# speechbrain/speechbrain

Measured on AMD Instinct MI355X. Metric: audio-sec/s decoded (node), Conformer-L beam=10, higher is better.
Workload: dtype f32

## Files before the change

speechbrain_amd/csrc/ctc_prefix.hip:

```cpp
#include "common.h"
#include "internal.h"

namespace {

constexpr float kNeg = sbk::kCtcNeg;
constexpr int kNegE = -(1 << 20);
constexpr int kHead = 24;

struct BF {
  float mg, mb;
  int eg, eb;
};

__device__ __forceinline__ float bf_log(float m, int e) {
  if (!(m > 0.0f)) return kNeg;
  const double v = ((double)e + (double)log2f(m)) * 0.69314718055994530942;
  return v < (double)kNeg ? kNeg : (float)v;
}
__device__ __forceinline__ void bf_exp(float x, float* m, int* e) {
  if (!(x > -1e19f)) {
    *m = 0.0f;
    *e = kNegE;
    return;
  }
  const double y = (double)x * 1.44269504088896340736;
  const double ip = floor(y);
  *m = exp2f((float)(y - ip));
  *e = (int)ip;
}

constexpr int kSeg = 32;
__device__ __host__ __forceinline__ int nseg_of(int T) { return (T + kSeg - 1) / kSeg; }
__device__ __host__ __forceinline__ int beam_pitch(int beam) { return 16 * ((beam + 15) / 16); }

template <typename Row>
__device__ __forceinline__ void build_segment_tables(Row row, int T, int lane, float* __restrict__ sg,
                                                     float* __restrict__ sb, int* __restrict__ se, int bp) {
  const int nseg = nseg_of(T);
  for (int s0 = 0; s0 < nseg; s0 += 2) {
    const int seg = s0 + (lane >> 5);
    const int t = seg * kSeg + (lane & 31);
    BF v{0.0f, 0.0f, kNegE, kNegE};
    if (seg < nseg && t < T) v = row(t);
    int e = max(v.mg > 0.0f ? v.eg : kNegE, v.mb > 0.0f ? v.eb : kNegE);
#pragma unroll
    for (int m = 16; m >= 1; m >>= 1) e = max(e, sbk::shfl_xor(e, m));
    if (seg < nseg && t < T) {
      sg[(size_t)t * bp] = sbk::fast_ldexp(v.mg, v.eg - e);
      sb[t] = sbk::fast_ldexp(v.mb, v.eb - e);
    }
    if (seg < nseg && (lane & 31) == 0) se[(size_t)seg * bp] = e;
  }
}

__global__ void __launch_bounds__(256) ctc_emissions_kernel(float* __restrict__ x, float* __restrict__ xb_log,
                                                            const int32_t* __restrict__ enc_len, int T, int V, int blank, int ldp) {
  const int b = blockIdx.y, t = blockIdx.x;
  float* row = x + ((size_t)b * T + t) * ldp;
  const bool pad = t >= enc_len[b];
  if (threadIdx.x == 0) xb_log[b * T + t] = pad ? (blank == 0 ? 0.0f : kNeg) : row[blank];
  __syncthreads();
  for (int c = threadIdx.x; c < V; c += 256) row[c] = pad ? (c == 0 ? 1.0f : 0.0f) : expf(row[c]);
}

__global__ void __launch_bounds__(256) ctc_init_kernel(const float* __restrict__ xb_log, BF* __restrict__ st,
                                                       float* __restrict__ sg, float* __restrict__ sb,
                                                       int* __restrict__ se, float* __restrict__ psi_prev, int T,
                                                       int beam) {
  SBK_DYN_LDS(float, cum);
  const int b = blockIdx.x;
  const int nseg = nseg_of(T);
  if (threadIdx.x == 0) {
    float c = 0.0f;
    for (int t = 0; t < T; ++t) {
      c += xb_log[b * T + t];
      cum[t] = c;
    }
  }
  __syncthreads();
  for (int t = threadIdx.x; t < T; t += 256) {
    BF v;
    bf_exp(cum[t], &v.mg, &v.eg);
    v.mb = v.mg;
    v.eb = v.eg;
    for (int j = 0; j < beam; ++j) st[((size_t)b * beam + j) * T + t] = v;
  }
  if (threadIdx.x < beam) psi_prev[b * beam + threadIdx.x] = 0.0f;
  __syncthreads();
  const int lane = threadIdx.x & 63, wave = threadIdx.x >> 6;
  for (int j = wave; j < beam; j += 4) {
    const size_t n = (size_t)b * beam + j;
    const BF* rowp = st + n * T;
    const int bp = beam_pitch(beam);
    build_segment_tables([&](int t) { return rowp[t]; }, T, lane, sg + (size_t)b * T * bp + j, sb + n * T,
                         se + (size_t)b * nseg * bp + j, bp);
  }
}

struct CtcStepArgs {
  const int32_t* last_tok;
  const int32_t* enc_len;
  int B, T, V, beam, prefix_len, blank, eos;
  float weight;
  int eos_floor;
  int use_eos_threshold;
  float eos_threshold, minus_inf;
  const int32_t* step_ptr;
  int min_steps;
  const int32_t* utt_min;
  int utt_beam, step;
  const int32_t* win;
  int window;
  int ldp;
};
__device__ __forceinline__ void ctc_frame_range(int prefix_len, int T, const int32_t* win, int window, int* start, int* end) {
// ... 109 lines not shown
      for (int q = 0; q < CH; ++q) cur[k][q] = nxt[k][q];
    if (cb + CH < u_end) fetch(nxt, cb + CH);
#pragma unroll
    for (int q = 0; q < CH; ++q) {
      const float4* row = reinterpret_cast<const float4*>(tab + (size_t)min(cb + q, u_end - 1) * BP);
      float g[NV * 4];
#pragma unroll
      for (int v = 0; v < NV; ++v) {
        const float4 t4 = row[v];
        g[4 * v] = t4.x; g[4 * v + 1] = t4.y; g[4 * v + 2] = t4.z; g[4 * v + 3] = t4.w;
      }
#pragma unroll
      for (int k = 0; k < TPT; ++k)
#pragma unroll
        for (int j = 0; j < NB; ++j) part[k][j] = fmaf(g[j], cur[k][q], part[k][j]);
    }
    if (((cb + CH) % kSeg) == 0 || cb + CH >= u_end) {
      const int* es = segs + (cb / kSeg) * BP;
#pragma unroll
      for (int k = 0; k < TPT; ++k)
#pragma unroll
        for (int j = 0; j < NB; ++j) {
          const int kx = sbk::frexp_exp(part[k][j]);
          const int ep = part[k][j] > 0.0f ? es[j] + kx : kNegE;
          const float mp = sbk::fast_ldexp(part[k][j], -kx);
          const int P2 = max(Eps[k][j], ep);
          mps[k][j] = sbk::fast_ldexp(mps[k][j], Eps[k][j] - P2) + sbk::fast_ldexp(mp, ep - P2);
          Eps[k][j] = P2;
          part[k][j] = 0.0f;
        }
    }
  }
#pragma unroll
  for (int k = 0; k < TPT; ++k) {
    if (!c_ok[k]) continue;
#pragma unroll
    for (int j = 0; j < NB; ++j) {
      if (j0 + j < a.beam) {
        const int n = b * a.beam + j0 + j;
        float psi = bf_log(mps[k][j], Eps[k][j]);
        if (c[k] == a.eos) {
          const BF s = st[(size_t)n * T + last_frame];
          psi = bf_log(s.mg, s.eg);
        }
        if (c[k] == a.blank && a.eos != a.blank) psi = kNeg;
        psi_out[(size_t)n * V + c[k]] = psi;
      }
    }
  }
}

__global__ void __launch_bounds__(64) ctc_same_token_kernel(CtcStepArgs a, const float* __restrict__ P,
                                                            const BF* __restrict__ st, const float* __restrict__ sb,
                                                            const int* __restrict__ se, float* __restrict__ psi_out) {
  const int n = blockIdx.x, lane = threadIdx.x;
  if (a.step_ptr) a.prefix_len = a.step_ptr[0];
  const int b = n / a.beam, c = a.last_tok[n];
  const int T = a.T, V = a.V, nseg = nseg_of(T);
  if (c == a.eos || c == a.blank || c < 0 || c >= V) return;
  int start, end;
  ctc_frame_range(a.prefix_len, T, a.win, a.window, &start, &end);
  end = ctc_clip_to_length(end, a.blank, a.enc_len[b]);
  const float* Pb = P + (size_t)b * T * a.ldp;
  float m = 0.0f;
  int E = kNegE;
  if (lane == 0 && a.prefix_len == 0 && start == 1 && Pb[c] > 0.0f) {
    m = Pb[c];
    E = 0;
  }
  for (int u = start - 1 + lane; u < end - 1; u += 64) {
    const float bt = a.win ? st[(size_t)n * T + u].mb : sb[(size_t)n * T + u];
    const float term = bt * Pb[(size_t)(u + 1) * a.ldp + c];
    const int k = sbk::frexp_exp(term);
    const int eb = a.win ? st[(size_t)n * T + u].eb : se[((size_t)b * nseg + u / kSeg) * beam_pitch(a.beam) + n % a.beam];
    const int et = term > 0.0f ? eb + k : kNegE;
    const float mt = sbk::fast_ldexp(term, -k);
    const int E2 = max(E, et);
    m = sbk::fast_ldexp(m, E - E2) + sbk::fast_ldexp(mt, et - E2);
    E = E2;
  }
  int Emax = E;
#pragma unroll
  for (int k = 32; k >= 1; k >>= 1) Emax = max(Emax, sbk::shfl_xor(Emax, k));
  float v = sbk::fast_ldexp(m, E - Emax);
  v = sbk::wave_sum(v);
  if (lane == 0) psi_out[(size_t)n * V + c] = bf_log(v, Emax);
}

__global__ void __launch_bounds__(256) ctc_combine_kernel(CtcStepArgs a, const float* __restrict__ am,
                                                          const float* __restrict__ am_max,
                                                          const float* __restrict__ psi,
                                                          const float* __restrict__ psi_prev, float* __restrict__ comb,
                                                          const float* __restrict__ extra) {
  const int n = blockIdx.y;
  const int c = blockIdx.x * 256 + threadIdx.x;
  if (c >= a.V) return;
  float v = am[(size_t)n * a.V + c];
  if (c == a.eos) {
    const int step = a.step_ptr ? a.step_ptr[0] : a.step;
    const bool floor = a.utt_min ? step < a.utt_min[n / a.utt_beam] : (a.step_ptr ? step < a.min_steps : a.eos_floor);
    if (floor) v = a.minus_inf;
    if (a.use_eos_threshold && !(v > a.eos_threshold * am_max[n])) v = a.minus_inf;
  }
  if (extra) v = sbk::add_rn(v, extra[(size_t)n * a.V + c]);
  if (c == a.blank) v = kNeg;
  comb[(size_t)n * a.V + c] = sbk::score_ctc(v, psi[(size_t)n * a.V + c], psi_prev[n], a.weight);
}

struct AMap {
  float a, c, d, v0, v1;
  int ea, ec, ed, e0, e1;
};
struct AState {
  float nb, bl;
  int e;
};
__device__ __forceinline__ int clamp_e(int e) { return max(e, kNegE); }
__device__ __forceinline__ void norm1(float& x, int& e) {
  const int k = sbk::frexp_exp(x);
  x = sbk::fast_ldexp(x, -k);
  e = x > 0.0f ? clamp_e(e + k) : kNegE;
}
__device__ __forceinline__ void norm2(float& x, float& y, int& e) {
  const float m = fmaxf(x, y);
  const int k = sbk::frexp_exp(m);
  x = sbk::fast_ldexp(x, -k);
  y = sbk::fast_ldexp(y, -k);
  e = m > 0.0f ? e + k : kNegE;
}
__device__ __forceinline__ void bf_add(float& x, int& ex, float y, int ey) {
  const int ax = x > 0.0f ? ex : kNegE, ay = y > 0.0f ? ey : kNegE;
  const int E = max(ax, ay);
// ... 36 lines not shown
  return r;
}
__device__ __forceinline__ AMap frame_map(float pc, float pb, float mphi, int ephi) {
  AMap m;
  m.a = pc;
  m.ea = 0;
  norm1(m.a, m.ea);
  m.c = pb;
  m.ec = 0;
  norm1(m.c, m.ec);
  m.d = m.c;
  m.ed = m.ec;
  m.v0 = m.a * mphi;
  m.e0 = clamp_e(m.ea + ephi);
  norm1(m.v0, m.e0);
  m.v1 = 0.0f;
  m.e1 = kNegE;
  return m;
}
__device__ __forceinline__ AMap identity_map() { return AMap{1.0f, 0.0f, 1.0f, 0.0f, 0.0f, 0, kNegE, 0, kNegE, kNegE}; }
__device__ __forceinline__ AMap shfl_up_map(const AMap& m, int delta, int lane) {
  const int src = max(lane - delta, 0);
  AMap r;
  r.a = sbk::shfl(m.a, src);
  r.c = sbk::shfl(m.c, src);
  r.d = sbk::shfl(m.d, src);
  r.v0 = sbk::shfl(m.v0, src);
  r.v1 = sbk::shfl(m.v1, src);
  r.ea = sbk::shfl(m.ea, src);
  r.ec = sbk::shfl(m.ec, src);
  r.ed = sbk::shfl(m.ed, src);
  r.e0 = sbk::shfl(m.e0, src);
  r.e1 = sbk::shfl(m.e1, src);
  return r;
}

struct CtcAdvArgs {
  const float* P;
  const BF* st_old;
  const float* psi;
  const int32_t* parent;
  const int32_t* token;
  const int32_t* parent_last_tok;
  BF* st_new;
  float* sg_new;
  float* sb_new;
  int* se_new;
  float* psi_prev_new;
  int n_bh, T, V, beam, prefix_len, blank;
  const int32_t* step_ptr;
  const int32_t* win;
  int window;
  int ldp;
};

__global__ void __launch_bounds__(64) ctc_advance_kernel(CtcAdvArgs a) {
  SBK_DYN_LDS(float, lds);
  if (a.step_ptr) a.prefix_len = a.step_ptr[0];
  const int T = a.T;
  float* pc = lds;
  float* pb = pc + T;
  float* mph = pb + T;
  int* eph = reinterpret_cast<int*>(mph + T);
  float* onb = reinterpret_cast<float*>(eph + T);
  float* obl = onb + T;
  int* oe = reinterpret_cast<int*>(obl + T);
  const int n = blockIdx.x, lane = threadIdx.x;
  const int b = n / a.beam, p = a.parent[n], c = a.token[n];
  const bool same = a.parent_last_tok[p] == c;
  const float* Pb = a.P + (size_t)b * T * a.ldp;
  for (int tb = 0; tb < T; tb += 256) {
    float vpc[4], vpb[4];
    BF vs[4];
#pragma unroll
    for (int u = 0; u < 4; ++u) {
      const int t = min(tb + u * 64 + lane, T - 1);
      vpc[u] = Pb[(size_t)t * a.ldp + c];
      vpb[u] = Pb[(size_t)t * a.ldp + a.blank];
      vs[u] = a.st_old[(size_t)p * T + t];
    }
#pragma unroll
    for (int u = 0; u < 4; ++u) {
      const int t = tb + u * 64 + lane;
      if (t < T) {
        pc[t] = vpc[u];
        pb[t] = vpb[u];
        mph[t] = same ? vs[u].mb : vs[u].mg;
        eph[t] = same ? vs[u].eb : vs[u].eg;
      }
    }
  }
  __syncthreads();
  {
    int start, end;
    ctc_frame_range(a.prefix_len, T, a.win, a.window, &start, &end);
    const bool first = a.prefix_len == 0 && pc[0] > 0.0f;
    AState r0{first ? pc[0] : 0.0f, 0.0f, first ? 0 : kNegE};
    norm2(r0.nb, r0.bl, r0.e);
    const AState zero{0.0f, 0.0f, kNegE};
    const AState s0 = start == 1 ? r0 : zero;
    for (int t = lane; t < T; t += 64)
      if (t < start || t >= end) {
        onb[t] = t == 0 ? r0.nb : 0.0f;
        obl[t] = 0.0f;
        oe[t] = t == 0 ? r0.e : kNegE;
      }
    const int nfr = max(end - start, 0);
    const int fpl = (nfr + 63) / 64;
    const int f0 = min(start + lane * fpl, end), f1 = min(f0 + fpl, end);
    AMap mine = identity_map();
    for (int t = f0; t < f1; ++t) mine = compose(frame_map(pc[t], pb[t], mph[t - 1], eph[t - 1]), mine);
#pragma unroll
    for (int dlt = 1; dlt < 64; dlt <<= 1) {
      const AMap other = shfl_up_map(mine, dlt, lane);
      if (lane >= dlt) mine = compose(mine, other);
    }
    AMap pre = shfl_up_map(mine, 1, lane);
    if (lane == 0) pre = identity_map();
    AState st = apply_map(pre, s0);
    for (int t = f0; t < f1; ++t) {
      st = apply_map(frame_map(pc[t], pb[t], mph[t - 1], eph[t - 1]), st);
      onb[t] = st.nb;
      obl[t] = st.bl;
      oe[t] = st.e;
    }
  }
  __syncthreads();
  BF* bfrow = reinterpret_cast<BF*>(pc);
  for (int t0 = 0; t0 < T; t0 += 64) {
    const int t = t0 + lane;
    BF s{0.0f, 0.0f, kNegE, kNegE};
    if (t < T) {
      const float g = onb[t] + obl[t];
      const int kg = sbk::frexp_exp(g), kb = sbk::frexp_exp(obl[t]);
      s.mg = g > 0.0f ? sbk::fast_ldexp(g, 1 - kg) : 0.0f;
      s.eg = g > 0.0f ? oe[t] + kg - 1 : kNegE;
      s.mb = obl[t] > 0.0f ? sbk::fast_ldexp(obl[t], 1 - kb) : 0.0f;
      s.eb = obl[t] > 0.0f ? oe[t] + kb - 1 : kNegE;
      a.st_new[(size_t)n * T + t] = s;
// ... 54 lines not shown
  if (threadIdx.x == 0) {
    const unsigned u = (prefix & 0x80000000u) ? (prefix & 0x7fffffffu) : ~prefix;
    thr[blockIdx.x] = __uint_as_float(u);
  }
}

__global__ void __launch_bounds__(256) ctc_partial_combine_kernel(float* __restrict__ comb, const float* __restrict__ thr,
                                                                  const float* __restrict__ psi,
                                                                  const float* __restrict__ psi_prev, int V, int blank,
                                                                  int eos, float weight, float minus_inf) {
  const int n = blockIdx.y;
  const int c = blockIdx.x * 256 + threadIdx.x;
  if (c >= V) return;
  const float base = comb[(size_t)n * V + c];
  float p = (base >= thr[n] || c == eos) ? psi[(size_t)n * V + c] : minus_inf;
  if (c == blank && eos != blank) p = minus_inf;
  comb[(size_t)n * V + c] = base + (p - psi_prev[n]) * weight;
}

__global__ void __launch_bounds__(256) row_max_kernel(const float* __restrict__ x, float* __restrict__ out, int V) {
  __shared__ float red[4];
  const float* xr = x + (size_t)blockIdx.x * V;
  float m = -INFINITY;
  for (int c = threadIdx.x; c < V; c += 256) m = fmaxf(m, xr[c]);
  m = sbk::wave_max(m);
  if ((threadIdx.x & 63) == 0) red[threadIdx.x >> 6] = m;
  __syncthreads();
  if (threadIdx.x == 0) out[blockIdx.x] = fmaxf(fmaxf(red[0], red[1]), fmaxf(red[2], red[3]));
}

}

namespace sbk {

namespace {
struct StateView {
  BF* st;
  float* sg;
  float* sb;
  int* se;
};
StateView view(float* base, int B, int beam, int T) {
  const size_t n_bh = (size_t)B * beam, bp = beam_pitch(beam);
  StateView v;
  v.st = reinterpret_cast<BF*>(base);
  v.sg = base + 4 * n_bh * T;
  v.sb = v.sg + (size_t)B * T * bp;
  v.se = reinterpret_cast<int*>(v.sb + n_bh * T);
  return v;
}
}

int ctc_psi_step(const float* P, const float* state, const int32_t* last_tok, const int32_t* enc_len, float* psi, int B,
                 int T, int V, int beam, int prefix_len, int blank, int eos, hipStream_t st, const int32_t* win, int window, int ldp);

size_t ctc_state_floats(int B, int beam, int T) {
  const size_t n_bh = (size_t)B * beam, bp = beam_pitch(beam);
  return 4 * n_bh * T + (size_t)B * T * bp + n_bh * T + (size_t)B * nseg_of(T) * bp + 16;
}

int ctc_prepare(float* x, float* xb_log, const int32_t* enc_len, float* state, float* psi_prev, int B, int T, int V,
                int beam, int blank, hipStream_t st, int ldp) {
  if (ldp < V) ldp = V;
  SBK_LAUNCH(ctc_emissions_kernel, dim3(T, B), dim3(256), 0, st, x, xb_log, enc_len, T, V, blank, ldp);
  int rc = launch_status("ctc_emissions");
  if (rc) return rc;
  StateView v = view(state, B, beam, T);
  if (hipMemsetAsync(v.sg, 0, (size_t)B * T * beam_pitch(beam) * sizeof(float), st) != hipSuccess) return fail(1, "ctc: memset");
  SBK_LAUNCH(ctc_init_kernel, dim3(B), dim3(256), (size_t)T * sizeof(float), st, (const float*)xb_log, v.st, v.sg, v.sb,
             v.se, psi_prev, T, beam);
  return launch_status("ctc_init");
}

int ctc_psi_step(const float* P, const float* state, const int32_t* last_tok, const int32_t* enc_len, float* psi, int B,
                 int T, int V, int beam, int prefix_len, int blank, int eos, hipStream_t st, const int32_t* win, int window, int ldp) {
  CtcStepArgs a{last_tok, enc_len, B, T, V, beam, prefix_len, blank, eos, 0.0f, 0, 0, 0.0f, 0.0f, g_step_ptr, 0};
  a.win = win;
  a.window = window;
  a.ldp = ldp < V ? V : ldp;
  const StateView v = view(const_cast<float*>(state), B, beam, T);
  ProfScope prof("ctc_score_step", 2.0 * B * beam * (double)T * V, 4.0 * B * (double)T * V + 4.0 * B * beam * V, st);
  constexpr int tpt = 1;
  dim3 grid(cdiv(V, 256 * tpt), B, beam_pitch(beam) / 16), block(256);
  const size_t lds = ((size_t)T * 16 + (size_t)((T + kSeg - 1) / kSeg) * 16) * sizeof(float);
  if (lds > 160 * 1024) return fail(SBK_EINVAL, "ctc_psi_step: T=%d frames need %zu B of LDS (max 160 KiB)", T, lds);
#define SBK_CTC_LAUNCH_NT(NB, TP, NT)                                                                                   \
  do {                                                                                                                  \
    if (allow_dyn_lds(ctc_score_step_kernel<NB, TP, NT>, lds) != hipSuccess)                                            \
      return fail(SBK_EINVAL, "ctc_psi_step: cannot raise the LDS window to %zu B", lds);                               \
    SBK_LAUNCH((ctc_score_step_kernel<NB, TP, NT>), grid, block, lds, st, a, P, (const BF*)v.st, (const float*)v.sg,    \
               (const int*)v.se, psi);                                                                                  \
  } while (0)
#define SBK_CTC_LAUNCH_ONE(NB, TP)                                                                                      \
  do {                                                                                                                  \
    if (g_nt_mask & 4)                                                                                                  \
      SBK_CTC_LAUNCH_NT(NB, TP, true);                                                                                  \
    else                                                                                                                \
      SBK_CTC_LAUNCH_NT(NB, TP, false);                                                                                 \
  } while (0)
#define SBK_CTC_LAUNCH(NB) SBK_CTC_LAUNCH_ONE(NB, 1)
  if (beam == 1) {
    SBK_CTC_LAUNCH(1);
  } else if (beam <= 4) {
    SBK_CTC_LAUNCH(4);
  } else if (beam <= 10) {
    SBK_CTC_LAUNCH(10);
  } else {
    SBK_CTC_LAUNCH(16);
  }
#undef SBK_CTC_LAUNCH
#undef SBK_CTC_LAUNCH_ONE
#undef SBK_CTC_LAUNCH_NT
  int rc = launch_status("ctc_score_step");
  if (rc) return rc;
  SBK_LAUNCH(ctc_same_token_kernel, dim3(B * beam), dim3(64), 0, st, a, P, (const BF*)v.st, (const float*)v.sb,
             (const int*)v.se, psi);
  return launch_status("ctc_same_token");
}

int ctc_combine(const float* am, const float* am_max, const float* psi, const float* psi_prev, float* comb, int n_bh,
                int V, int blank, int eos, float weight, int eos_floor, int use_thr, float thr, float minus_inf,
                const float* extra, hipStream_t st, const int32_t* utt_min, int beam, int step) {
  CtcStepArgs a{nullptr, nullptr, 0, 0, V, 0, 0, blank, eos, weight, eos_floor, use_thr, thr, minus_inf, g_step_ptr,
                g_step_min_steps, utt_min, beam > 0 ? beam : 1, step};
  SBK_LAUNCH(ctc_combine_kernel, dim3(cdiv(V, 256), n_bh), dim3(256), 0, st, a, am, am_max, psi, psi_prev, comb, extra);
  return launch_status("ctc_combine");
}

int ctc_advance(const float* P, const float* state_old, const float* psi, const int32_t* parent, const int32_t* token,
                const int32_t* parent_last_tok, float* state_new, float* psi_prev_new, int n_bh, int T, int V, int beam,
                int prefix_len, int blank, hipStream_t st, const int32_t* win, int window, int ldp) {
  const StateView vo = view(const_cast<float*>(state_old), n_bh / beam, beam, T);
  const StateView vn = view(state_new, n_bh / beam, beam, T);
  CtcAdvArgs a{P, vo.st, psi, parent, token, parent_last_tok, vn.st, vn.sg, vn.sb, vn.se, psi_prev_new, n_bh, T, V, beam,
               prefix_len, blank, g_step_ptr, win, window, ldp < V ? V : ldp};
  const size_t lds = (size_t)7 * T * sizeof(float);
  if (lds > 64 * 1024) return fail(SBK_EINVAL, "ctc_advance: T=%d too long for the LDS window", T);
  ProfScope prof("ctc_advance", 14.0 * n_bh * T, 64.0 * n_bh * T, st);
  SBK_LAUNCH(ctc_advance_kernel, dim3(n_bh), dim3(64), lds, st, a);
  return launch_status("ctc_advance");
}

int am_only(const float* am, float* comb, int n_bh, int V, int eos, int eos_floor, int use_thr, float thr,
            float minus_inf, const float* am_max, const float* extra, hipStream_t st, const int32_t* utt_min, int beam,
            int step) {
  const int32_t* sp = g_step_ptr;
  const int min_steps = g_step_min_steps;
  SBK_LAUNCH(am_only_kernel, dim3(cdiv(V, 256), n_bh), dim3(256), 0, st, am, comb, V, eos, eos_floor, use_thr, thr,
             minus_inf, am_max, extra, sp, min_steps, utt_min, beam > 0 ? beam : 1, step);
  return launch_status("am_only");
}

int ctc_partial_combine(float* comb, float* thr, const float* psi, const float* psi_prev, int n_bh, int V, int k, int blank,
                        int eos, float weight, float minus_inf, hipStream_t st) {
  const int kk = k < 1 ? 1 : (k > V ? V : k);
  SBK_LAUNCH(row_kth_largest_kernel, dim3(n_bh), dim3(256), 0, st, (const float*)comb, thr, V, kk);
  SBK_LAUNCH(ctc_partial_combine_kernel, dim3(cdiv(V, 256), n_bh), dim3(256), 0, st, comb, (const float*)thr, psi, psi_prev,
             V, blank, eos, weight, minus_inf);
  return launch_status("ctc_partial_combine");
}

int row_max(const float* x, float* out, int rows, int V, hipStream_t st) {
  SBK_LAUNCH(row_max_kernel, dim3(rows), dim3(256), 0, st, x, out, V);
  return launch_status("row_max");
}

}


namespace {
__global__ void __launch_bounds__(256) ctc_score_delta_kernel(const float* __restrict__ psi, const float* __restrict__ psi_prev,
                                                              float* __restrict__ out, int V) {
  const int n = blockIdx.y, c = blockIdx.x * 256 + threadIdx.x;
  if (c < V) out[(size_t)n * V + c] = sbk::sub_rn(psi[(size_t)n * V + c], psi_prev[n]);
}
struct ScorerWs {
  float* phi[2];
  float* psi;
  float* psi_prev[2];
  float* xb;
};
size_t scorer_ws_floats(int B, int T, int V, int beam) {
  auto up = [](size_t n) { return (n + 63) & ~(size_t)63; };
  return 2 * up(sbk::ctc_state_floats(B, beam, T)) + up((size_t)B * beam * V) + 2 * up((size_t)B * beam) + up((size_t)B * T);
}
ScorerWs carve_scorer(void* ws, int B, int T, int V, int beam) {
  auto up = [](size_t n) { return (n + 63) & ~(size_t)63; };
  float* p = static_cast<float*>(ws);
  ScorerWs w;
  w.phi[0] = p, p += up(sbk::ctc_state_floats(B, beam, T));
  w.phi[1] = p, p += up(sbk::ctc_state_floats(B, beam, T));
  w.psi = p, p += up((size_t)B * beam * V);
  w.psi_prev[0] = p, p += up((size_t)B * beam);
  w.psi_prev[1] = p, p += up((size_t)B * beam);
  w.xb = p;
  return w;
}
}

extern "C" size_t sbk_ctc_scorer_workspace_bytes(int B, int T, int V, int beam) {
  if (B <= 0 || T <= 0 || V <= 0 || beam <= 0) return 0;
  return scorer_ws_floats(B, T, V, beam) * sizeof(float);
}

extern "C" int sbk_ctc_scorer_reset_f32(float* x, const int32_t* enc_len, void* ws, size_t ws_bytes, int B, int T, int V, int beam,
                                        int blank, sbk_stream_t stream) {
  if (B == 0) return 0;
  SBK_REQUIRE(x && enc_len && ws && B > 0 && T > 0 && V > 0 && beam > 0 && blank >= 0 && blank < V, "ctc_scorer_reset: bad arguments");
  SBK_REQUIRE(ws_bytes >= sbk_ctc_scorer_workspace_bytes(B, T, V, beam) && sbk::aligned16(ws) && sbk::aligned16(x),
              "ctc_scorer_reset: workspace too small (%zu B) or unaligned", ws_bytes);
  hipStream_t st = sbk::as_stream(stream);
  const ScorerWs w = carve_scorer(ws, B, T, V, beam);
  if (hipMemsetAsync(w.phi[1], 0, sbk::ctc_state_floats(B, beam, T) * sizeof(float), st) != hipSuccess)
    return sbk::fail(1, "ctc_scorer_reset: memset");
  return sbk::ctc_prepare(x, w.xb, enc_len, w.phi[0], w.psi_prev[0], B, T, V, beam, blank, st, V);
}

extern "C" int sbk_ctc_scorer_score_f32(const float* x, const int32_t* enc_len, void* ws, size_t ws_bytes, const int32_t* inp_tokens,
                                        int step, const int32_t* attn_window, int ctc_window_size, float* scores, int B, int T, int V,
                                        int beam, int blank, int eos, sbk_stream_t stream) {
  if (B == 0) return 0;
  SBK_REQUIRE(x && enc_len && ws && inp_tokens && scores && B > 0 && T > 0 && V > 0 && beam > 0 && step >= 0, "ctc_scorer_score: bad arguments");
  SBK_REQUIRE(ws_bytes >= sbk_ctc_scorer_workspace_bytes(B, T, V, beam), "ctc_scorer_score: workspace too small");
  SBK_REQUIRE(ctc_window_size >= 0 && (ctc_window_size == 0 || attn_window), "ctc_scorer_score: a window needs the {min, max} attention peaks");
  hipStream_t st = sbk::as_stream(stream);
  const ScorerWs w = carve_scorer(ws, B, T, V, beam);
  const int cur = step & 1;
  const int32_t* win = ctc_window_size > 0 ? attn_window : nullptr;
  int rc = sbk::ctc_psi_step(x, w.phi[cur], inp_tokens, enc_len, w.psi, B, T, V, beam, step, blank, eos, st, win, ctc_window_size, V);
  if (rc) return rc;
  SBK_LAUNCH(ctc_score_delta_kernel, dim3(sbk::cdiv(V, 256), B * beam), dim3(256), 0, st, (const float*)w.psi,
             (const float*)w.psi_prev[cur], scores, V);
  return sbk::launch_status("ctc_score_delta");
}

extern "C" int sbk_ctc_scorer_permute_f32(const float* x, void* ws, size_t ws_bytes, const int32_t* parent, const int32_t* token,
                                          const int32_t* parent_last_tok, int step, const int32_t* attn_window, int ctc_window_size,
                                          int B, int T, int V, int beam, int blank, sbk_stream_t stream) {
  if (B == 0) return 0;
  SBK_REQUIRE(x && ws && parent && token && parent_last_tok && B > 0 && T > 0 && V > 0 && beam > 0 && step >= 0, "ctc_scorer_permute: bad arguments");
  SBK_REQUIRE(ws_bytes >= sbk_ctc_scorer_workspace_bytes(B, T, V, beam), "ctc_scorer_permute: workspace too small");
  SBK_REQUIRE(ctc_window_size >= 0 && (ctc_window_size == 0 || attn_window), "ctc_scorer_permute: a window needs the {min, max} attention peaks");
  const ScorerWs w = carve_scorer(ws, B, T, V, beam);
  const int cur = step & 1;
  return sbk::ctc_advance(x, w.phi[cur], w.psi, parent, token, parent_last_tok, w.phi[cur ^ 1], w.psi_prev[cur ^ 1], B * beam, T, V,
                          beam, step, blank, sbk::as_stream(stream), ctc_window_size > 0 ? attn_window : nullptr, ctc_window_size, V);
}

extern "C" int sbk_prof_ctc_psi_repeat_f32(float* P_logsoftmax, const int32_t* enc_len, const int32_t* last_tok,
                                           float* psi, float* work, int B, int T, int V, int beam, int prefix_len,
                                           int iters, float* us_per_launch, sbk_stream_t stream) {
  SBK_REQUIRE(P_logsoftmax && enc_len && last_tok && psi && work && us_per_launch && iters > 0, "psi_repeat: bad arguments");
  hipStream_t st = sbk::as_stream(stream);
  float* state = work;
  float* xb = work + sbk::ctc_state_floats(B, beam, T);
  float* psi_prev = xb + (size_t)B * T;
  int rc = sbk::ctc_prepare(P_logsoftmax, xb, enc_len, state, psi_prev, B, T, V, beam, 0, st, V);
  hipEvent_t e0, e1;
  if (hipEventCreate(&e0) != hipSuccess || hipEventCreate(&e1) != hipSuccess) return sbk::fail(1, "event create");
  for (int i = 0; i < 2 && !rc; ++i)
    rc = sbk::ctc_psi_step(P_logsoftmax, state, last_tok, enc_len, psi, B, T, V, beam, prefix_len, 0, 2, st, nullptr, 0, V);
  (void)hipEventRecord(e0, st);
  for (int i = 0; i < iters && !rc; ++i)
    rc = sbk::ctc_psi_step(P_logsoftmax, state, last_tok, enc_len, psi, B, T, V, beam, prefix_len, 0, 2, st, nullptr, 0, V);
  (void)hipEventRecord(e1, st);
  (void)hipEventSynchronize(e1);
  float ms = 0.0f;
  (void)hipEventElapsedTime(&ms, e0, e1);
  *us_per_launch = ms * 1000.0f / iters;
  return rc;
}
```

speechbrain_amd/csrc/internal.h:

```cpp
#pragma once
#include "common.h"
#include "device.h"
#include "knobs.h"

namespace sbk {
int sk_route(int M, int N, int K, int* bt = nullptr);
int gemm_nt(const float* A, int lda, const float* W, int ldw, const float* bias, const float* R, int ldr, float* C,
            int ldc, int M, int N, int K, int act, float alpha, const int32_t* seq_len, int rows_per_seq,
            hipStream_t st);
int gemm_nt_x3(const float* A, int lda, const uint16_t* W3, const float* bias, const float* R, int ldr, float* C, int ldc,
               int M, int N, int K, int act, float alpha, const int32_t* seq_len, int rows_per_seq, hipStream_t st);
bool x3_routed(int M, int N, int K);
int gemm_nt_x3p(const uint16_t* PA, const uint16_t* PW, const float* bias, const float* R, int ldr, float* C, int ldc,
                uint16_t* PC, int M, int N, int K, int act, float alpha, const int32_t* seq_len, int rows_per_seq, hipStream_t st);
int gemm_nt_x3r(const float* A, int lda, const uint16_t* PW, const float* bias, const float* R, int ldr, float* C, int ldc, int M,
                int N, int K, int act, float alpha, hipStream_t st);
bool x3r_routed(int M, int N, int K);
int gemm_ln_nt_x3r(const float* A, int lda, const uint16_t* PWf, const float* bf, const float* R, int ldr, float* C, int ldc, int M,
                   int N, int K, float eps, int act, float alpha, hipStream_t st);
bool x3r_ln_routed(int K);
bool persist_eligible(const sbk_decoder_weights* W, int n, int B, int beam, int Lmax);
int persist_barriers(int n_layers);
int decoder_step_persist(const sbk_decoder_weights* W, const int32_t* tokens, const int32_t* kv_slot, const int32_t* enc_len,
                         float* x, float* qkv, float* ctx, float* q, float* ff, float* h, float* logits, float* const* kcache,
                         float* const* vcache, float* const* ckv, int* bar, int bar_seq, int* grid_io, int step, int n, int B, int T,
                         int beam, int Lmax, bool want_logits, hipStream_t st);
extern thread_local const int32_t* g_step_ptr;
extern thread_local int g_step_min_steps;
struct Lp256Args {
  const unsigned char* A;
  const unsigned char* W;
  const float* sa;
  const float* sw;
  const float* bias;
  const float* R;
  float* C;
  unsigned short* Cb;
  unsigned char* C8;
  float c8_scale;
  long lda, ldw;
  int ldr, ldc, ldcb, ldc8, M, N, act;
  float alpha;
  int KT, tiles_m, tiles_n, tiles, whole;
};
bool lp256_routed(const Lp256Args& a);
int gemm_nt_lp256(const Lp256Args& a, bool fp8, hipStream_t st);
constexpr float kCtcNeg = -1e20f;
__device__ __forceinline__ float ls_logit(float x, float b1, float b2, float inv_temp) {
  return mul_rn(add_rn(add_rn(x, b1), b2), inv_temp);
}
__device__ __forceinline__ float ls_out(float v, float lse, float w) { return mul_rn(w, sub_rn(v, lse)); }
__device__ __forceinline__ float score_ctc(float v, float psi, float psi_prev, float weight) {
  return add_rn(v, mul_rn(sub_rn(psi, psi_prev), weight));
}
__device__ __forceinline__ float score_cand(float seq, float comb, float norm) {
  const float x = add_rn(seq, comb);
  return norm > 0.0f ? x / norm : x;
}
int embed_pos(const int32_t* tok, const float* emb, const float* pe_row, float* x, int n, int d, float scale,
              hipStream_t st);
int self_attn_step(const float* qkv, float* kcache, float* vcache, const int32_t* kv_slot, float* out, int n, int d,
                   int H, int step, int nslot, int Lmax, hipStream_t st, const int32_t* key_tok = nullptr,
                   int key_stride = 0, int key_shift = 0, int key_first = 0, int pad_idx = 0, int group = 1);
int cross_attn_step(const float* q, const float* kv, const int32_t* enc_len, float* out, float* part, int B, int T,
                    int d, int H, int beam, hipStream_t st);
size_t cross_attn_partial_floats(int B, int T, int H, int Dh, int beam);
int log_softmax_rows(const float* x, float* out, int rows, int V, float temperature, float weight, hipStream_t st,
                     const float* bias = nullptr, const float* bias2 = nullptr, int ld = 0);
int ctc_prepare(float* x, float* xb_log, const int32_t* enc_len, float* state, float* psi_prev, int B, int T, int V,
                int beam, int blank, hipStream_t st, int ldp = 0);
size_t ctc_state_floats(int B, int beam, int T);
int ctc_psi_step(const float* P, const float* state, const int32_t* last_tok, const int32_t* enc_len, float* psi, int B,
                 int T, int V, int beam, int prefix_len, int blank, int eos, hipStream_t st, const int32_t* win = nullptr,
                 int window = 0, int ldp = 0);
int cross_attn_avg_probs(const float* q, const float* kv, const int32_t* enc_len, float* out, int n, int T, int d, int H,
                         int beam, hipStream_t st);
int ctc_combine(const float* am, const float* am_max, const float* psi, const float* psi_prev, float* comb, int n_bh,
                int V, int blank, int eos, float weight, int eos_floor, int use_thr, float thr, float minus_inf,
                const float* extra, hipStream_t st, const int32_t* utt_min = nullptr, int beam = 1, int step = 0);
int ctc_advance(const float* x, const float* phi_old, const float* psi, const int32_t* parent, const int32_t* token,
                const int32_t* parent_last_tok, float* phi_new, float* psi_prev_new, int n_bh, int T, int V, int beam,
                int prefix_len, int blank, hipStream_t st, const int32_t* win = nullptr, int window = 0, int ldp = 0);
int am_only(const float* am, float* comb, int n_bh, int V, int eos, int eos_floor, int use_thr, float thr,
            float minus_inf, const float* am_max, const float* extra, hipStream_t st, const int32_t* utt_min = nullptr,
            int beam = 1, int step = 0);
int row_max(const float* x, float* out, int rows, int V, hipStream_t st);
int ctc_partial_combine(float* comb, float* thr, const float* psi, const float* psi_prev, int n_bh, int V, int k, int blank,
                        int eos, float weight, float minus_inf, hipStream_t st);
int gemm_nt_ws(const float* A, int lda, const float* W, int ldw, const float* bias, const float* R, int ldr, float* C,
               int ldc, int M, int N, int K, int act, float alpha, const int32_t* seq_len, int rows_per_seq, float* ws,
               size_t ws_floats, hipStream_t st);
int gemm_ln_nt(const float* A, int lda, const float* Wf, int ldw, const float* bf, const float* R, int ldr, float* C,
               int ldc, int M, int N, int K, float eps, int act, float alpha, hipStream_t st);
int layernorm(const float* x, const float* gamma, const float* beta, float* y, int rows, int d, float eps, int act,
              hipStream_t st);
int relpos_attention(const float* qkv, const float* pos, const float* bias_u, const float* bias_v,
                     const int32_t* key_len, float* out, float* attn, int B, int T, int H, int Dh, float scale,
                     hipStream_t st, int chunk = 0, int left = -1);
int glu_dwconv(const float* h, const float* w, const float* bias, float* y, int B, int T, int d, int ksize,
               hipStream_t st, int chunk = 0);
}
```

speechbrain_amd/native.py:

```python

from __future__ import annotations

import collections
import contextlib
import ctypes
import math
import os
import threading
import weakref
from ctypes import POINTER, c_char_p, c_float, c_int, c_int32, c_void_p
from typing import Optional

import torch

_HERE = os.path.dirname(os.path.abspath(__file__))
LIB_PATH = os.path.join(_HERE, "csrc", "libsbk_hip.so")

ACT_NONE, ACT_SWISH, ACT_GELU, ACT_RELU, ACT_LEAKY_RELU = 0, 1, 2, 3, 4

_lib = None


class SbkError(RuntimeError):
    pass
# ... 1648 lines not shown
    nbytes = lib.sbk_greedy_search_workspace_bytes(ctypes.byref(handle.W), B, T, max_steps)
    ws = _Workspace(nbytes, dev)
    out_tok = torch.zeros(B, L, dtype=torch.int32, device=dev)
    out_sc = torch.zeros(B, L, dtype=torch.float32, device=dev)
    flag = _host_flag(dev)
    steps = c_int32(0)
    _chk(lib.sbk_greedy_search_f32(ctypes.byref(handle.W), _p(enc), _p(enc_len), ws.ptr, nbytes,
                                   _p(out_tok), _p(out_sc), c_void_p(flag.data_ptr()), ctypes.byref(steps), B, T,
                                   int(min_steps), int(max_steps), int(bos), int(eos), int(check_every), _stream(enc)),
         "sbk_greedy_search_f32")
    return out_tok, out_sc, steps.value


def prompted_greedy_search(handle: DecoderHandle, enc, enc_len, prompt, max_new, eos, logit_bias=None, first_bias=None,
                           probe=None, check_every=8):
    lib = load()
    _dev_ok(enc, enc_len, prompt, logit_bias, first_bias)
    B, T, _ = enc.shape
    P = prompt.shape[1]
    dev = enc.device
    L = max(int(max_new), 1)
    handle.ready.wait(enc.device)
    nbytes = lib.sbk_prompted_greedy_search_workspace_bytes(ctypes.byref(handle.W), B, T, P, int(max_new))
    ws = _Workspace(nbytes, dev)
    out_tok = torch.zeros(B, L, dtype=torch.int32, device=dev)
    out_sc = torch.zeros(B, L, dtype=torch.float32, device=dev)
    out_probe = torch.zeros(B, dtype=torch.float32, device=dev) if probe is not None else None
    flag = _host_flag(dev)
    steps = c_int32(0)
    _chk(lib.sbk_prompted_greedy_search_f32(
        ctypes.byref(handle.W), _p(enc), _p(enc_len), _p(prompt), P, _p(logit_bias), _p(first_bias),
        ws.ptr, nbytes, _p(out_tok), _p(out_sc), int(probe[0]) if probe else 0,
        int(probe[1]) if probe else 0, _p(out_probe), c_void_p(flag.data_ptr()), ctypes.byref(steps), B, T, int(max_new),
        int(eos), int(check_every), _stream(enc)), "sbk_prompted_greedy_search_f32")
    return out_tok, out_sc, steps.value, out_probe


def decoder_prefix(handle: DecoderHandle, tokens, enc, enc_len):
    lib = load()
    _dev_ok(tokens, enc, enc_len)
    n, L = tokens.shape
    T = enc.shape[1]
    handle.ready.wait(enc.device)
    nbytes = lib.sbk_decoder_prefix_workspace_bytes(ctypes.byref(handle.W), n, T, L)
    ws = _Workspace(nbytes, enc.device)
    pred = torch.empty(n, L, handle.W.d_model, dtype=torch.float32, device=enc.device)
    _chk(lib.sbk_decoder_prefix_f32(ctypes.byref(handle.W), _p(tokens), _p(enc), _p(enc_len), ws.ptr, nbytes, _p(pred), n, T, L,
                                    _stream(enc)), "sbk_decoder_prefix_f32")
    return pred


class CTCStepScorer:

    def __init__(self, log_probs, enc_len, blank, eos, ctc_window_size=0):
        _dev_ok(log_probs, enc_len)
        _f32(log_probs)
        self.x, self.enc_len = log_probs, enc_len.to(torch.int32)
        self.B, self.T, self.V = log_probs.shape
        self.blank, self.eos, self.window = int(blank), int(eos), int(ctc_window_size)
        self.beam, self.ws, self.nbytes = 0, None, 0

    def _ready(self, beam):
        if self.beam == beam:
            return
        if self.beam:
            raise SbkError(f"CTCStepScorer: the beam width changed from {self.beam} to {beam} inside one utterance batch")
        lib = load()
        self.beam = beam
        self.nbytes = lib.sbk_ctc_scorer_workspace_bytes(self.B, self.T, self.V, beam)
        self.ws = _Workspace(self.nbytes, self.x.device)
        _chk(lib.sbk_ctc_scorer_reset_f32(_p(self.x), _p(self.enc_len), self.ws.ptr, self.nbytes, self.B,
                                          self.T, self.V, beam, self.blank, _stream(self.x)), "sbk_ctc_scorer_reset_f32")

    def score(self, inp_tokens, step, attn_window=None):
        n = inp_tokens.shape[0]
        if n % self.B:
            raise SbkError(f"CTCStepScorer: {n} hypotheses for {self.B} utterances")
        self._ready(n // self.B)
        tok = inp_tokens.to(torch.int32).contiguous()
        out = torch.empty(n, self.V, dtype=torch.float32, device=self.x.device)
        _chk(load().sbk_ctc_scorer_score_f32(_p(self.x), _p(self.enc_len), self.ws.ptr, self.nbytes, _p(tok),
                                             int(step), _p(attn_window), self.window if attn_window is not None else 0, _p(out), self.B,
                                             self.T, self.V, self.beam, self.blank, self.eos, _stream(self.x)), "sbk_ctc_scorer_score_f32")
        return out

    def permute(self, parent, token, parent_last_tok, step, attn_window=None):
        par, tk, last = (t.to(torch.int32).contiguous() for t in (parent, token, parent_last_tok))
        _chk(load().sbk_ctc_scorer_permute_f32(_p(self.x), self.ws.ptr, self.nbytes, _p(par), _p(tk), _p(last),
                                               int(step), _p(attn_window), self.window if attn_window is not None else 0, self.B, self.T,
                                               self.V, self.beam, self.blank, _stream(self.x)), "sbk_ctc_scorer_permute_f32")


def log_softmax(x, temperature=1.0, weight=1.0):
    lib = load()
    V = x.shape[-1]
    x2 = x.reshape(-1, V)
    _dev_ok(x2)
    out = torch.empty_like(x)
    _chk(lib.sbk_log_softmax_f32(_p(x2), _p(out), x2.shape[0], V, float(temperature), float(weight), _stream(x2)),
         "sbk_log_softmax_f32")
    return out


def _rel_len(rel_len, device):
    return None if rel_len is None else rel_len.to(device=device, dtype=torch.float32).contiguous()


def ctc_greedy_decode(x, rel_len, blank):
    lib = load()
    _f32(x)
    B, T, V = x.shape
    x = x.contiguous()
    rel = _rel_len(rel_len, x.device)
    _dev_ok(x, rel)
    tokens = torch.empty(B, T, dtype=torch.int32, device=x.device)
    count = torch.empty(B, dtype=torch.int32, device=x.device)
    _chk(lib.sbk_ctc_greedy_decode_f32(_p(x), _p(rel), _p(tokens), _p(count), B, T, V, int(blank), _stream(x)),
         "sbk_ctc_greedy_decode_f32")
    return tokens, count


def ctc_beam_search(x, rel_len, table, n_vocab, cfg, lm=None):
# ... 177 lines not shown
```

Baseline: 13210.

## Add token-major transposed CTC emission copy for same-token and advance kernels

After the emissions are exponentiated, a tiled transpose kernel writes a token-major copy (B x V x padded T) into the scorer workspace. The same-token kernel then reads a contiguous time column per token with an unrolled batch of loads, and the advance kernel loads the token and blank columns with 16-byte vector loads instead of strided per-frame gathers. This costs extra workspace memory and a one-time transpose per utterance batch in exchange for coalesced per-step reads. The old strided path is kept as a fallback when the workspace is too small.

```diff
diff --git a/speechbrain_amd/csrc/ctc_prefix.hip b/speechbrain_amd/csrc/ctc_prefix.hip
--- a/speechbrain_amd/csrc/ctc_prefix.hip
+++ b/speechbrain_amd/csrc/ctc_prefix.hip
@@ -61,6 +61,30 @@
   if (threadIdx.x == 0) xb_log[b * T + t] = pad ? (blank == 0 ? 0.0f : kNeg) : row[blank];
   __syncthreads();
   for (int c = threadIdx.x; c < V; c += 256) row[c] = pad ? (c == 0 ? 1.0f : 0.0f) : expf(row[c]);
+}
+
+constexpr int kTrTile = 64;
+__device__ __host__ __forceinline__ int ctc_tp(int T) { return (T + 31) & ~31; }
+__global__ void __launch_bounds__(256) ctc_transpose_kernel(const float* __restrict__ P, float* __restrict__ Pt, int T, int V,
+                                                            int ldp, int Tp) {
+  __shared__ float tile[kTrTile][kTrTile + 1];
+  const int b = blockIdx.z, t0 = blockIdx.x * kTrTile, c0 = blockIdx.y * kTrTile;
+  const int lane = threadIdx.x & 63, wave = threadIdx.x >> 6;
+  const float* Pb = P + (size_t)b * T * ldp;
+  const int c = c0 + lane;
+  float v[kTrTile / 4];
+#pragma unroll
+  for (int i = 0; i < kTrTile / 4; ++i) v[i] = Pb[(size_t)min(t0 + 4 * i + wave, T - 1) * ldp + min(c, V - 1)];
+#pragma unroll
+  for (int i = 0; i < kTrTile / 4; ++i) tile[4 * i + wave][lane] = (t0 + 4 * i + wave < T && c < V) ? v[i] : 0.0f;
+  __syncthreads();
+  float* Ptb = Pt + (size_t)b * V * Tp;
+  const int t = t0 + lane;
+#pragma unroll
+  for (int i = 0; i < kTrTile / 4; ++i) {
+    const int cr = c0 + 4 * i + wave;
+    if (cr < V && t < Tp) Ptb[(size_t)cr * Tp + t] = tile[lane][4 * i + wave];
+  }
 }
 
 __global__ void __launch_bounds__(256) ctc_init_kernel(const float* __restrict__ xb_log, BF* __restrict__ st,
@@ -276,7 +300,8 @@
 
 __global__ void __launch_bounds__(64) ctc_same_token_kernel(CtcStepArgs a, const float* __restrict__ P,
                                                             const BF* __restrict__ st, const float* __restrict__ sb,
-                                                            const int* __restrict__ se, float* __restrict__ psi_out) {
+                                                            const int* __restrict__ se, float* __restrict__ psi_out,
+                                                            const float* __restrict__ Pt, int Tp) {
   const int n = blockIdx.x, lane = threadIdx.x;
   if (a.step_ptr) a.prefix_len = a.step_ptr[0];
   const int b = n / a.beam, c = a.last_tok[n];
@@ -288,20 +313,52 @@
   const float* Pb = P + (size_t)b * T * a.ldp;
   float m = 0.0f;
   int E = kNegE;
-  if (lane == 0 && a.prefix_len == 0 && start == 1 && Pb[c] > 0.0f) {
-    m = Pb[c];
-    E = 0;
-  }
-  for (int u = start - 1 + lane; u < end - 1; u += 64) {
-    const float bt = a.win ? st[(size_t)n * T + u].mb : sb[(size_t)n * T + u];
-    const float term = bt * Pb[(size_t)(u + 1) * a.ldp + c];
-    const int k = sbk::frexp_exp(term);
-    const int eb = a.win ? st[(size_t)n * T + u].eb : se[((size_t)b * nseg + u / kSeg) * beam_pitch(a.beam) + n % a.beam];
-    const int et = term > 0.0f ? eb + k : kNegE;
-    const float mt = sbk::fast_ldexp(term, -k);
-    const int E2 = max(E, et);
-    m = sbk::fast_ldexp(m, E - E2) + sbk::fast_ldexp(mt, et - E2);
-    E = E2;
+  if (Pt) {
+    constexpr int kSameRun = 8;
+    const float* Pc = Pt + ((size_t)b * V + c) * Tp;
+    if (lane == 0 && a.prefix_len == 0 && start == 1 && Pc[0] > 0.0f) {
+      m = Pc[0];
+      E = 0;
+    }
+    const int u_end = end - 1;
+    for (int base = start - 1; base < u_end; base += 64 * kSameRun) {
+      float pv[kSameRun], bt[kSameRun];
+      int eb[kSameRun];
+#pragma unroll
+      for (int i = 0; i < kSameRun; ++i) {
+        const int u = min(base + 64 * i + lane, u_end - 1);
+        pv[i] = Pc[u + 1];
+        bt[i] = a.win ? st[(size_t)n * T + u].mb : sb[(size_t)n * T + u];
+        eb[i] = a.win ? st[(size_t)n * T + u].eb : se[((size_t)b * nseg + u / kSeg) * beam_pitch(a.beam) + n % a.beam];
+      }
+#pragma unroll
+      for (int i = 0; i < kSameRun; ++i) {
+        if (base + 64 * i + lane >= u_end) continue;
+        const float term = bt[i] * pv[i];
+        const int k = sbk::frexp_exp(term);
+        const int et = term > 0.0f ? eb[i] + k : kNegE;
+        const float mt = sbk::fast_ldexp(term, -k);
+        const int E2 = max(E, et);
+        m = sbk::fast_ldexp(m, E - E2) + sbk::fast_ldexp(mt, et - E2);
+        E = E2;
+      }
+    }
+  } else {
+    if (lane == 0 && a.prefix_len == 0 && start == 1 && Pb[c] > 0.0f) {
+      m = Pb[c];
+      E = 0;
+    }
+    for (int u = start - 1 + lane; u < end - 1; u += 64) {
+      const float bt = a.win ? st[(size_t)n * T + u].mb : sb[(size_t)n * T + u];
+      const float term = bt * Pb[(size_t)(u + 1) * a.ldp + c];
+      const int k = sbk::frexp_exp(term);
+      const int eb = a.win ? st[(size_t)n * T + u].eb : se[((size_t)b * nseg + u / kSeg) * beam_pitch(a.beam) + n % a.beam];
+      const int et = term > 0.0f ? eb + k : kNegE;
+      const float mt = sbk::fast_ldexp(term, -k);
+      const int E2 = max(E, et);
+      m = sbk::fast_ldexp(m, E - E2) + sbk::fast_ldexp(mt, et - E2);
+      E = E2;
+    }
   }
   int Emax = E;
 #pragma unroll
@@ -444,6 +501,8 @@
   const int32_t* win;
   int window;
   int ldp;
+  const float* Pt;
+  int Tp;
 };
 
 __global__ void __launch_bounds__(64) ctc_advance_kernel(CtcAdvArgs a) {
@@ -461,22 +520,36 @@
   const int b = n / a.beam, p = a.parent[n], c = a.token[n];
   const bool same = a.parent_last_tok[p] == c;
   const float* Pb = a.P + (size_t)b * T * a.ldp;
+  const bool tm = a.Pt != nullptr;
+  const float* gc = tm ? a.Pt + ((size_t)b * a.V + c) * a.Tp : nullptr;
+  const float* gb = tm ? a.Pt + ((size_t)b * a.V + a.blank) * a.Tp : nullptr;
   for (int tb = 0; tb < T; tb += 256) {
-    float vpc[4], vpb[4];
+    float vpc[4] = {0.0f, 0.0f, 0.0f, 0.0f}, vpb[4] = {0.0f, 0.0f, 0.0f, 0.0f};
     BF vs[4];
+    const int t4 = tb + 4 * lane;
+    if (tm) {
+      const int tq = min(t4, a.Tp - 4);
+      const float4 vc = sbk::ld16<false>(gc + tq), vb = sbk::ld16<false>(gb + tq);
+      vpc[0] = vc.x, vpc[1] = vc.y, vpc[2] = vc.z, vpc[3] = vc.w;
+      vpb[0] = vb.x, vpb[1] = vb.y, vpb[2] = vb.z, vpb[3] = vb.w;
+    }
 #pragma unroll
     for (int u = 0; u < 4; ++u) {
       const int t = min(tb + u * 64 + lane, T - 1);
-      vpc[u] = Pb[(size_t)t * a.ldp + c];
-      vpb[u] = Pb[(size_t)t * a.ldp + a.blank];
+      if (!tm) {
+        vpc[u] = Pb[(size_t)t * a.ldp + c];
+        vpb[u] = Pb[(size_t)t * a.ldp + a.blank];
+      }
       vs[u] = a.st_old[(size_t)p * T + t];
     }
 #pragma unroll
     for (int u = 0; u < 4; ++u) {
-      const int t = tb + u * 64 + lane;
+      const int t = tb + u * 64 + lane, te = tm ? t4 + u : t;
+      if (te < T) {
+        pc[te] = vpc[u];
+        pb[te] = vpb[u];
+      }
       if (t < T) {
-        pc[t] = vpc[u];
-        pb[t] = vpb[u];
         mph[t] = same ? vs[u].mb : vs[u].mg;
         eph[t] = same ? vs[u].eb : vs[u].eg;
       }
@@ -637,19 +710,29 @@
 }
 
 int ctc_psi_step(const float* P, const float* state, const int32_t* last_tok, const int32_t* enc_len, float* psi, int B,
-                 int T, int V, int beam, int prefix_len, int blank, int eos, hipStream_t st, const int32_t* win, int window, int ldp);
+                 int T, int V, int beam, int prefix_len, int blank, int eos, hipStream_t st, const int32_t* win, int window, int ldp, const float* Pt);
 
 size_t ctc_state_floats(int B, int beam, int T) {
   const size_t n_bh = (size_t)B * beam, bp = beam_pitch(beam);
   return 4 * n_bh * T + (size_t)B * T * bp + n_bh * T + (size_t)B * nseg_of(T) * bp + 16;
 }
 
+size_t ctc_pt_floats(int B, int T, int V) { return (size_t)B * V * ctc_tp(T); }
+
 int ctc_prepare(float* x, float* xb_log, const int32_t* enc_len, float* state, float* psi_prev, int B, int T, int V,
-                int beam, int blank, hipStream_t st, int ldp) {
+                int beam, int blank, hipStream_t st, int ldp, float* Pt) {
   if (ldp < V) ldp = V;
   SBK_LAUNCH(ctc_emissions_kernel, dim3(T, B), dim3(256), 0, st, x, xb_log, enc_len, T, V, blank, ldp);
   int rc = launch_status("ctc_emissions");
   if (rc) return rc;
+  if (Pt) {
+    const int Tp = ctc_tp(T);
+    ProfScope prof("ctc_transpose", 0.0, 4.0 * B * (double)V * (T + Tp), st);
+    SBK_LAUNCH(ctc_transpose_kernel, dim3(cdiv(Tp, kTrTile), cdiv(V, kTrTile), B), dim3(256), 0, st, (const float*)x, Pt, T, V,
+               ldp, Tp);
+    rc = launch_status("ctc_transpose");
+    if (rc) return rc;
+  }
   StateView v = view(state, B, beam, T);
   if (hipMemsetAsync(v.sg, 0, (size_t)B * T * beam_pitch(beam) * sizeof(float), st) != hipSuccess) return fail(1, "ctc: memset");
   SBK_LAUNCH(ctc_init_kernel, dim3(B), dim3(256), (size_t)T * sizeof(float), st, (const float*)xb_log, v.st, v.sg, v.sb,
@@ -658,7 +741,7 @@
 }
 
 int ctc_psi_step(const float* P, const float* state, const int32_t* last_tok, const int32_t* enc_len, float* psi, int B,
-                 int T, int V, int beam, int prefix_len, int blank, int eos, hipStream_t st, const int32_t* win, int window, int ldp) {
+                 int T, int V, int beam, int prefix_len, int blank, int eos, hipStream_t st, const int32_t* win, int window, int ldp, const float* Pt) {
   CtcStepArgs a{last_tok, enc_len, B, T, V, beam, prefix_len, blank, eos, 0.0f, 0, 0, 0.0f, 0.0f, g_step_ptr, 0};
   a.win = win;
   a.window = window;
@@ -699,7 +782,7 @@
   int rc = launch_status("ctc_score_step");
   if (rc) return rc;
   SBK_LAUNCH(ctc_same_token_kernel, dim3(B * beam), dim3(64), 0, st, a, P, (const BF*)v.st, (const float*)v.sb,
-             (const int*)v.se, psi);
+             (const int*)v.se, psi, Pt, ctc_tp(T));
   return launch_status("ctc_same_token");
 }
 
@@ -714,11 +797,11 @@
 
 int ctc_advance(const float* P, const float* state_old, const float* psi, const int32_t* parent, const int32_t* token,
                 const int32_t* parent_last_tok, float* state_new, float* psi_prev_new, int n_bh, int T, int V, int beam,
-                int prefix_len, int blank, hipStream_t st, const int32_t* win, int window, int ldp) {
+                int prefix_len, int blank, hipStream_t st, const int32_t* win, int window, int ldp, const float* Pt) {
   const StateView vo = view(const_cast<float*>(state_old), n_bh / beam, beam, T);
   const StateView vn = view(state_new, n_bh / beam, beam, T);
   CtcAdvArgs a{P, vo.st, psi, parent, token, parent_last_tok, vn.st, vn.sg, vn.sb, vn.se, psi_prev_new, n_bh, T, V, beam,
-               prefix_len, blank, g_step_ptr, win, window, ldp < V ? V : ldp};
+               prefix_len, blank, g_step_ptr, win, window, ldp < V ? V : ldp, Pt, ctc_tp(T)};
   const size_t lds = (size_t)7 * T * sizeof(float);
   if (lds > 64 * 1024) return fail(SBK_EINVAL, "ctc_advance: T=%d too long for the LDS window", T);
   ProfScope prof("ctc_advance", 14.0 * n_bh * T, 64.0 * n_bh * T, st);
@@ -764,12 +847,14 @@
   float* psi;
   float* psi_prev[2];
   float* xb;
+  float* pt;
 };
-size_t scorer_ws_floats(int B, int T, int V, int beam) {
+size_t scorer_ws_floats(int B, int T, int V, int beam, bool with_pt) {
   auto up = [](size_t n) { return (n + 63) & ~(size_t)63; };
-  return 2 * up(sbk::ctc_state_floats(B, beam, T)) + up((size_t)B * beam * V) + 2 * up((size_t)B * beam) + up((size_t)B * T);
-}
-ScorerWs carve_scorer(void* ws, int B, int T, int V, int beam) {
+  return 2 * up(sbk::ctc_state_floats(B, beam, T)) + up((size_t)B * beam * V) + 2 * up((size_t)B * beam) + up((size_t)B * T) +
+         (with_pt ? up(sbk::ctc_pt_floats(B, T, V)) : 0);
+}
+ScorerWs carve_scorer(void* ws, size_t ws_bytes, int B, int T, int V, int beam) {
   auto up = [](size_t n) { return (n + 63) & ~(size_t)63; };
   float* p = static_cast<float*>(ws);
   ScorerWs w;
@@ -778,27 +863,31 @@
   w.psi = p, p += up((size_t)B * beam * V);
   w.psi_prev[0] = p, p += up((size_t)B * beam);
   w.psi_prev[1] = p, p += up((size_t)B * beam);
-  w.xb = p;
+  w.xb = p, p += up((size_t)B * T);
+  w.pt = ws_bytes >= scorer_ws_floats(B, T, V, beam, true) * sizeof(float) ? p : nullptr;
   return w;
 }
 }
 
 extern "C" size_t sbk_ctc_scorer_workspace_bytes(int B, int T, int V, int beam) {
   if (B <= 0 || T <= 0 || V <= 0 || beam <= 0) return 0;
-  return scorer_ws_floats(B, T, V, beam) * sizeof(float);
+  return scorer_ws_floats(B, T, V, beam, true) * sizeof(float);
+}
+static bool scorer_ws_fits(size_t ws_bytes, int B, int T, int V, int beam) {
+  return ws_bytes >= scorer_ws_floats(B, T, V, beam, false) * sizeof(float);
 }
 
 extern "C" int sbk_ctc_scorer_reset_f32(float* x, const int32_t* enc_len, void* ws, size_t ws_bytes, int B, int T, int V, int beam,
                                         int blank, sbk_stream_t stream) {
   if (B == 0) return 0;
   SBK_REQUIRE(x && enc_len && ws && B > 0 && T > 0 && V > 0 && beam > 0 && blank >= 0 && blank < V, "ctc_scorer_reset: bad arguments");
-  SBK_REQUIRE(ws_bytes >= sbk_ctc_scorer_workspace_bytes(B, T, V, beam) && sbk::aligned16(ws) && sbk::aligned16(x),
+  SBK_REQUIRE(scorer_ws_fits(ws_bytes, B, T, V, beam) && sbk::aligned16(ws) && sbk::aligned16(x),
               "ctc_scorer_reset: workspace too small (%zu B) or unaligned", ws_bytes);
   hipStream_t st = sbk::as_stream(stream);
-  const ScorerWs w = carve_scorer(ws, B, T, V, beam);
+  const ScorerWs w = carve_scorer(ws, ws_bytes, B, T, V, beam);
   if (hipMemsetAsync(w.phi[1], 0, sbk::ctc_state_floats(B, beam, T) * sizeof(float), st) != hipSuccess)
     return sbk::fail(1, "ctc_scorer_reset: memset");
-  return sbk::ctc_prepare(x, w.xb, enc_len, w.phi[0], w.psi_prev[0], B, T, V, beam, blank, st, V);
+  return sbk::ctc_prepare(x, w.xb, enc_len, w.phi[0], w.psi_prev[0], B, T, V, beam, blank, st, V, w.pt);
 }
 
 extern "C" int sbk_ctc_scorer_score_f32(const float* x, const int32_t* enc_len, void* ws, size_t ws_bytes, const int32_t* inp_tokens,
@@ -806,13 +895,14 @@
                                         int beam, int blank, int eos, sbk_stream_t stream) {
   if (B == 0) return 0;
   SBK_REQUIRE(x && enc_len && ws && inp_tokens && scores && B > 0 && T > 0 && V > 0 && beam > 0 && step >= 0, "ctc_scorer_score: bad arguments");
-  SBK_REQUIRE(ws_bytes >= sbk_ctc_scorer_workspace_bytes(B, T, V, beam), "ctc_scorer_score: workspace too small");
+  SBK_REQUIRE(scorer_ws_fits(ws_bytes, B, T, V, beam), "ctc_scorer_score: workspace too small");
   SBK_REQUIRE(ctc_window_size >= 0 && (ctc_window_size == 0 || attn_window), "ctc_scorer_score: a window needs the {min, max} attention peaks");
   hipStream_t st = sbk::as_stream(stream);
-  const ScorerWs w = carve_scorer(ws, B, T, V, beam);
+  const ScorerWs w = carve_scorer(ws, ws_bytes, B, T, V, beam);
   const int cur = step & 1;
   const int32_t* win = ctc_window_size > 0 ? attn_window : nullptr;
-  int rc = sbk::ctc_psi_step(x, w.phi[cur], inp_tokens, enc_len, w.psi, B, T, V, beam, step, blank, eos, st, win, ctc_window_size, V);
+  int rc = sbk::ctc_psi_step(x, w.phi[cur], inp_tokens, enc_len, w.psi, B, T, V, beam, step, blank, eos, st, win, ctc_window_size, V,
+                             w.pt);
   if (rc) return rc;
   SBK_LAUNCH(ctc_score_delta_kernel, dim3(sbk::cdiv(V, 256), B * beam), dim3(256), 0, st, (const float*)w.psi,
              (const float*)w.psi_prev[cur], scores, V);
@@ -824,12 +914,13 @@
                                           int B, int T, int V, int beam, int blank, sbk_stream_t stream) {
   if (B == 0) return 0;
   SBK_REQUIRE(x && ws && parent && token && parent_last_tok && B > 0 && T > 0 && V > 0 && beam > 0 && step >= 0, "ctc_scorer_permute: bad arguments");
-  SBK_REQUIRE(ws_bytes >= sbk_ctc_scorer_workspace_bytes(B, T, V, beam), "ctc_scorer_permute: workspace too small");
+  SBK_REQUIRE(scorer_ws_fits(ws_bytes, B, T, V, beam), "ctc_scorer_permute: workspace too small");
   SBK_REQUIRE(ctc_window_size >= 0 && (ctc_window_size == 0 || attn_window), "ctc_scorer_permute: a window needs the {min, max} attention peaks");
-  const ScorerWs w = carve_scorer(ws, B, T, V, beam);
+  const ScorerWs w = carve_scorer(ws, ws_bytes, B, T, V, beam);
   const int cur = step & 1;
   return sbk::ctc_advance(x, w.phi[cur], w.psi, parent, token, parent_last_tok, w.phi[cur ^ 1], w.psi_prev[cur ^ 1], B * beam, T, V,
-                          beam, step, blank, sbk::as_stream(stream), ctc_window_size > 0 ? attn_window : nullptr, ctc_window_size, V);
+                          beam, step, blank, sbk::as_stream(stream), ctc_window_size > 0 ? attn_window : nullptr, ctc_window_size, V,
+                          w.pt);
 }
 
 extern "C" int sbk_prof_ctc_psi_repeat_f32(float* P_logsoftmax, const int32_t* enc_len, const int32_t* last_tok,
diff --git a/speechbrain_amd/csrc/internal.h b/speechbrain_amd/csrc/internal.h
--- a/speechbrain_amd/csrc/internal.h
+++ b/speechbrain_amd/csrc/internal.h
@@ -68,11 +68,12 @@
 int log_softmax_rows(const float* x, float* out, int rows, int V, float temperature, float weight, hipStream_t st,
                      const float* bias = nullptr, const float* bias2 = nullptr, int ld = 0);
 int ctc_prepare(float* x, float* xb_log, const int32_t* enc_len, float* state, float* psi_prev, int B, int T, int V,
-                int beam, int blank, hipStream_t st, int ldp = 0);
+                int beam, int blank, hipStream_t st, int ldp = 0, float* Pt = nullptr);
 size_t ctc_state_floats(int B, int beam, int T);
+size_t ctc_pt_floats(int B, int T, int V);
 int ctc_psi_step(const float* P, const float* state, const int32_t* last_tok, const int32_t* enc_len, float* psi, int B,
                  int T, int V, int beam, int prefix_len, int blank, int eos, hipStream_t st, const int32_t* win = nullptr,
-                 int window = 0, int ldp = 0);
+                 int window = 0, int ldp = 0, const float* Pt = nullptr);
 int cross_attn_avg_probs(const float* q, const float* kv, const int32_t* enc_len, float* out, int n, int T, int d, int H,
                          int beam, hipStream_t st);
 int ctc_combine(const float* am, const float* am_max, const float* psi, const float* psi_prev, float* comb, int n_bh,
@@ -80,7 +81,8 @@
                 const float* extra, hipStream_t st, const int32_t* utt_min = nullptr, int beam = 1, int step = 0);
 int ctc_advance(const float* x, const float* phi_old, const float* psi, const int32_t* parent, const int32_t* token,
                 const int32_t* parent_last_tok, float* phi_new, float* psi_prev_new, int n_bh, int T, int V, int beam,
-                int prefix_len, int blank, hipStream_t st, const int32_t* win = nullptr, int window = 0, int ldp = 0);
+                int prefix_len, int blank, hipStream_t st, const int32_t* win = nullptr, int window = 0, int ldp = 0,
+                const float* Pt = nullptr);
 int am_only(const float* am, float* comb, int n_bh, int V, int eos, int eos_floor, int use_thr, float thr,
             float minus_inf, const float* am_max, const float* extra, hipStream_t st, const int32_t* utt_min = nullptr,
             int beam = 1, int step = 0);
diff --git a/speechbrain_amd/native.py b/speechbrain_amd/native.py
--- a/speechbrain_amd/native.py
+++ b/speechbrain_amd/native.py
@@ -1724,13 +1724,14 @@
 
 class CTCStepScorer:
 
-    def __init__(self, log_probs, enc_len, blank, eos, ctc_window_size=0):
+    def __init__(self, log_probs, enc_len, blank, eos, ctc_window_size=0, token_major=True):
         _dev_ok(log_probs, enc_len)
         _f32(log_probs)
         self.x, self.enc_len = log_probs, enc_len.to(torch.int32)
         self.B, self.T, self.V = log_probs.shape
         self.blank, self.eos, self.window = int(blank), int(eos), int(ctc_window_size)
         self.beam, self.ws, self.nbytes = 0, None, 0
+        self.token_major = bool(token_major)
 
     def _ready(self, beam):
         if self.beam == beam:
@@ -1740,6 +1741,8 @@
         lib = load()
         self.beam = beam
         self.nbytes = lib.sbk_ctc_scorer_workspace_bytes(self.B, self.T, self.V, beam)
+        if not self.token_major:
+            self.nbytes -= 4 * ((self.B * self.V * ((self.T + 31) & ~31) + 63) & ~63)
         self.ws = _Workspace(self.nbytes, self.x.device)
         _chk(lib.sbk_ctc_scorer_reset_f32(_p(self.x), _p(self.enc_len), self.ws.ptr, self.nbytes, self.B,
                                           self.T, self.V, beam, self.blank, _stream(self.x)), "sbk_ctc_scorer_reset_f32")
```

Measured after the change: 13030. 0.986x the previous value.
